# intuitive-robots/mdt_policy

Hardware: AMD Instinct MI355X
Metric: action-chunks/sec (10-step denoise, horizon=10) (higher is better)
Workload: dtype f32

## Files before the change

### include/mdt_hip_ops.h

```cpp
#ifndef MDT_HIP_OPS_H
#define MDT_HIP_OPS_H

#include <stdint.h>
#include "mdt_hip.h"

#ifdef __cplusplus
extern "C" {
#endif

enum { MDT_ACT_NONE = 0, MDT_ACT_GELU = 1, MDT_ACT_MISH = 2, MDT_ACT_SILU = 3,
       MDT_ACT_SWIGLU = 4  };
enum { MDT_HEAD_DENOISED = 0, MDT_HEAD_DDIM = 1, MDT_HEAD_RAW = 2,
       MDT_HEAD_PLAN = 3  };

int64_t mdt_op_packed_numel(int64_t N, int64_t K);

mdt_status mdt_op_pack_weight(const float *w, int64_t n_rows, int64_t K, float *packed, int64_t n_off,
                              int64_t N_total, void *stream);
mdt_status mdt_op_pack_weight_glu(const float *w, int64_t H2, int64_t K, float *packed, void *stream);

typedef struct {
    const float *A;
    int64_t lda;
    const float *Wp;
    const float *bias;
    float *out;
    int64_t ldo;
    int32_t M, N, K;
    int32_t ln;
    const float *ln_w, *ln_b;
    const float *mod;
    int64_t mod_stride;
    int32_t shift_off, scale_off;
    int32_t rows_per_sample;
    int32_t act;
    int32_t residual;
    int32_t gate_off;
    int32_t gin, gout, goff;
    const float *rowvec;
    int32_t batch;
    int64_t bs_a, bs_w, bs_out;
    const float *aux;
    int32_t aux_mode;
    int32_t a_parts;
    int64_t a_part_stride;
    float *a_merged;
    const void *Wp_split;
} mdt_gemm_args;

mdt_status mdt_op_gemm(const mdt_gemm_args *args, void *stream);

mdt_status mdt_op_mlp(const mdt_gemm_args *fc, const mdt_gemm_args *proj, float *parts, int64_t part_stride,
                      int32_t *n_parts, void *stream);
mdt_status mdt_op_pack_weight_split(const float *w, int64_t n_rows, int64_t K, void *image, void *stream);
mdt_status mdt_op_pack_weight_split_rows(const float *w, int64_t n_rows, int64_t K, void *image, int64_t n_off, void *stream);
mdt_status mdt_op_mlp_split(const mdt_gemm_args *fc, const mdt_gemm_args *proj, const void *fc_split, const void *proj_split,
                            float *parts, int64_t part_stride, int32_t *n_parts, void *stream);
void mdt_op_set_mlp_split(int32_t on);
void mdt_op_set_mlp_fuse_min(int32_t rows);
void mdt_op_set_side_jobs(int32_t on);
int64_t mdt_op_side_jobs_paired(void);
void mdt_op_trace_mlp(int32_t enable);
int32_t mdt_op_trace_mlp_read(float *us, int32_t cap);
int32_t mdt_op_trace_mlp_read_empty(float *us, int32_t cap);
mdt_status mdt_op_clock_stamp(uint64_t *out16, void *stream);
void mdt_op_set_ws_split(int32_t on);

void mdt_op_set_mlp_skew(int32_t v);

void mdt_op_set_gemm_geometry(int32_t geometry);

typedef struct {
    const float *q; int64_t ldq;
    const float *k; const float *v;
    int64_t ldkv;
    float *out; int64_t ldo;
    int32_t B, H, hd, Tq, Tk;
    int32_t causal;
    int32_t rope;
} mdt_attn_args;

mdt_status mdt_op_attention(const mdt_attn_args *args, void *stream);

mdt_status mdt_op_attn_proj(const mdt_gemm_args *proj, const float *qkv, int64_t ldq, int32_t hd, int32_t T, int32_t causal,
                            void *stream);
void mdt_op_set_attn_wide_min(int32_t rows);

mdt_status mdt_op_layernorm(const float *in, const float *w, const float *b, float *out, int64_t M, int32_t D,
                            void *stream);

typedef struct {
    const float *y;
    const float *ln_w;
    const float *ln_b;
    const float *Wp, *bp;
    const float *x;
    const float *sigma;
    int64_t sigma_stride;
    float *out;
    int32_t M, D, A, rows_per_sample;
    int32_t mode;
    const float *step;
    float sigma_data;
    float *y_next;
    const float *Wa, *ba;
    int32_t no_ln;
    int32_t y_parts;
    int64_t y_part_stride;
} mdt_head_args;

mdt_status mdt_op_head(const mdt_head_args *args, void *stream);

typedef struct {
    const float *kv; int64_t ldkv;
    const float *WqT_p;
    const float *bq;
    const float *Wo_p;
    float *U, *Wf;
    float *c;
    int32_t B, H, hd, D, Te;
} mdt_xfold_args;
// ... 26 lines not shown
```

### mdt_policy_amd/_lib.py

```python
from __future__ import annotations

import ctypes as C
import os
import threading

from . import build as _build

c_float_p = C.POINTER(C.c_float)


class MDTHipError(RuntimeError):
    def __init__(self, status: int, message: str):
        super().__init__(f"libmdt_hip status {status}: {message}")
        self.status = status


class MDTConfig(C.Structure):
    _fields_ = [(n, C.c_int32) for n in (
        "arch", "embed_dim", "n_heads", "n_enc_layers", "n_dec_layers", "action_dim", "obs_dim", "goal_dim",
        "n_obs_token", "goal_seq_len", "action_seq_len", "use_mlp_goal", "use_modality_encoder", "use_abs_pos_emb",
        "use_rot_embed", "use_ada_conditioning", "use_noise_encoder", "linear_output", "bias")] + [
        ("sigma_data", C.c_float), ("no_goal_conditioning", C.c_int32), ("proprio_dim", C.c_int32),
        ("use_proprio", C.c_int32)]

# ... 155 lines not shown
_VP, _I32, _I64, _F = C.c_void_p, C.c_int32, C.c_int64, C.c_float
SYMBOLS = [
    ("mdt_last_error", C.c_char_p, []),
    ("mdt_version", C.c_char_p, []),
    ("mdt_set_allocator", _I32, [_VP, _VP, _VP]),
    ("mdt_allocator_detach", _I32, []),
    ("mdt_create", _I32, [C.POINTER(MDTConfig), C.POINTER(_VP)]),
    ("mdt_destroy", _I32, [_VP]),
    ("mdt_param_count", _I64, [_VP]),
    ("mdt_param_name", C.c_char_p, [_VP, _I64]),
    ("mdt_param_numel", _I64, [_VP, _I64]),
    ("mdt_load_param", _I32, [_VP, C.c_char_p, _VP, _I64, _VP]),
    ("mdt_load_params", _I32, [_VP, _I32, C.POINTER(C.c_char_p), C.POINTER(C.c_void_p), C.POINTER(_I64), _VP]),
    ("mdt_reserve", _I32, [_VP, _I64]),
    ("mdt_ws_generation", _I64, [_VP]),
    ("mdt_encode", _I32, [_VP, _VP, _VP, _VP, _I32, _I32, _VP, _I64, _VP, _VP]),
    ("mdt_denoise_cached", _I32, [_VP, _VP, _VP, _I64, _I32, _VP, _VP]),
    ("mdt_forward", _I32, [_VP, _VP, _VP, _VP, _I32, _VP, _VP, _I64, _VP, _VP, _VP]),
    ("mdt_sample_ddim", _I32, [_VP, _VP, _VP, _VP, _I32, _VP, C.POINTER(C.c_float), _I32, _I64, _VP, _VP, _VP]),
    ("mdt_sample_ddim_dev", _I32, [_VP, _VP, _VP, _VP, _I32, _VP, _VP, _I32, _I64, _VP, _VP, _VP]),
    ("mdt_sample", _I32, [_VP, _VP, _VP, _VP, _I32, _VP, _I32, C.POINTER(SamplerParams), C.POINTER(C.c_float), _I32, _VP, _I32,
                          _I64, _VP, _VP, _VP]),
    ("mdt_sample_dev", _I32, [_VP, _VP, _VP, _VP, _I32, _VP, _I32, C.POINTER(SamplerParams), _VP, _I32, _VP, _I32, _I64, _VP,
                              _VP, _VP]),
    ("mdt_sampler_plan", _I32, [_I32, C.POINTER(SamplerParams), C.POINTER(C.c_float), _I32, C.POINTER(SamplerPlan)]),
    ("mdt_sample_dpm_adaptive", _I32, [_VP, _VP, _VP, _VP, _I32, _VP, C.c_float, C.c_float, C.POINTER(DpmAdaptiveParams), _I64,
                                       _VP, _VP, C.POINTER(DpmAdaptiveInfo), _VP]),
    ("mdt_dpm_control_init", _I32, [C.POINTER(DpmControl)] + [C.c_double] * 6),
    ("mdt_dpm_control_update", _I32, [C.POINTER(DpmControl), C.c_float, C.POINTER(C.c_int32)]),
    ("mdt_dpm_adaptive_plan", _I32, [_I32, C.c_float, C.c_float, C.POINTER(SamplerPlan)]),
    ("mdt_op_trace_mlp", None, [_I32]),
    ("mdt_op_trace_mlp_read", _I32, [_VP, _I32]),
    ("mdt_op_trace_mlp_read_empty", _I32, [_VP, _I32]),
    ("mdt_op_clock_stamp", _I32, [_VP, _VP]),
    ("mdt_op_set_ws_split", None, [_I32]),
    ("mdt_op_set_tn_split", None, [_I32]),
    ("mdt_loss_fwd", _I32, [_VP, _VP, _VP, _VP, _I32, _VP, _VP, _VP, _I64, _VP, _VP, _VP, _VP]),
    ("mdt_flops_per_chunk", C.c_double, [_VP, _I32]),
    ("mdt_fnv1_32", C.c_uint32, [C.c_char_p, C.c_uint64, C.c_uint32]),
    ("mdt_op_packed_numel", _I64, [_I64, _I64]),
    ("mdt_op_pack_weight", _I32, [_VP, _I64, _I64, _VP, _I64, _I64, _VP]),
    ("mdt_op_pack_weight_glu", _I32, [_VP, _I64, _I64, _VP, _VP]),
    ("mdt_op_gemm", _I32, [C.POINTER(GemmArgs), _VP]),
    ("mdt_op_mlp", _I32, [C.POINTER(GemmArgs), C.POINTER(GemmArgs), _VP, _I64, C.POINTER(_I32), _VP]),
    ("mdt_op_pack_weight_split", _I32, [_VP, _I64, _I64, _VP, _VP]),
    ("mdt_op_pack_weight_split_rows", _I32, [_VP, _I64, _I64, _VP, _I64, _VP]),
    ("mdt_op_mlp_split", _I32, [C.POINTER(GemmArgs), C.POINTER(GemmArgs), _VP, _VP, _VP, _I64, C.POINTER(_I32), _VP]),
    ("mdt_op_set_mlp_split", None, [_I32]),
    ("mdt_op_set_gemm_geometry", None, [_I32]),
    ("mdt_op_set_mlp_fuse_min", None, [_I32]),
    ("mdt_op_set_side_jobs", None, [_I32]),
    ("mdt_op_side_jobs_paired", _I64, []),
    ("mdt_op_set_mlp_skew", None, [_I32]),
    ("mdt_op_set_attn_wide_min", None, [_I32]),
    ("mdt_op_attention", _I32, [C.POINTER(AttnArgs), _VP]),
    ("mdt_op_attn_proj", _I32, [C.POINTER(GemmArgs), _VP, _I64, _I32, _I32, _I32, _VP]),
    ("mdt_op_xattn_fold", _I32, [C.POINTER(XFoldArgs), _VP]),
    ("mdt_op_xattn_apply", _I32, [C.POINTER(XApplyArgs), _VP]),
    ("mdt_op_attn_xattn", _I32, [C.POINTER(GemmArgs), _VP, _I64, C.POINTER(XApplyArgs), _I32, _I32, _VP]),
    ("mdt_op_xattn_gemm", _I32, [C.POINTER(XApplyArgs), C.POINTER(GemmArgs), _VP]),
    ("mdt_op_layernorm", _I32, [_VP, _VP, _VP, _VP, _I64, _I32, _VP]),
    ("mdt_op_head", _I32, [C.POINTER(HeadArgs), _VP]),
    ("mdt_op_action_embed", _I32, [_VP, _VP, _I64, _F, _VP, _VP, _VP, _I64, _I32, _I32, _I32, _VP]),
    ("mdt_train_prepare", _I32, [_VP]),
    ("mdt_grad_numel", _I64, [_VP]),
    ("mdt_grad_offset", _I64, [_VP, _I64]),
    ("mdt_train_loss_fwd", _I32, [_VP, _VP, _VP, _VP, _I32, _VP, _VP, _VP, _I64, C.POINTER(Dropout), _VP, _VP, _VP,
                                  C.POINTER(_I32), _VP]),
    ("mdt_train_loss_bwd", _I32, [_VP, _I32, _VP, _VP, _VP, _VP, _VP, _VP, _VP]),
    ("mdt_train_loss_bwd_stages", _I32, [_VP]),
    ("mdt_train_loss_bwd_stage", _I32, [_VP, _I32, _I32, _VP, _VP, _VP, _VP, _VP, _VP, _VP]),
    ("mdt_train_param_stage", _I32, [_VP, _I64]),
    ("mdt_train_encode_fwd", _I32, [_VP, _VP, _VP, _VP, _I32, _I32, _VP, _I64, C.POINTER(Dropout), _VP, C.POINTER(_I32),
                                    _VP]),
    ("mdt_train_encode_bwd", _I32, [_VP, _I32, _VP, _VP, _VP, _VP, _VP, _VP]),
    ("mdt_tape_release", _I32, [_VP, _I32]),
    ("mdt_denoise_vjp", _I32, [_VP, _VP, _VP, _VP, _I32, _VP, _VP, _VP, _I64, _VP, _VP, _VP]),
    ("mdt_op_pack_weight_t", _I32, [_VP, _I64, _I64, _I64, _VP, _I64, _I64, _VP]),
    ("mdt_op_pack_many", _I32, [_I32, C.POINTER(C.c_void_p), C.POINTER(_I32), C.POINTER(_I32), C.POINTER(C.c_void_p),
                                C.POINTER(C.c_void_p), _VP]),
    ("mdt_op_ln_fwd_train", _I32, [C.POINTER(LnTrainArgs), _VP]),
    ("mdt_op_ln_bwd", _I32, [C.POINTER(LnBwdArgs), _VP]),
    ("mdt_op_attn_bwd", _I32, [C.POINTER(AttnBwdArgs), _VP]),
    ("mdt_op_act_fwd", _I32, [_VP, _VP, _I64, _I32, _VP]),
    ("mdt_op_act_bwd", _I32, [_VP, _VP, _VP, _I64, _I32, _VP]),
    ("mdt_op_attn_fwd_train", _I32, [C.POINTER(AttnTrainArgs), _VP]),
    ("mdt_op_merge_fwd", _I32, [C.POINTER(MergeArgs), _VP]),
    ("mdt_op_merge_bwd", _I32, [C.POINTER(MergeArgs), _VP]),
    ("mdt_op_merge_ln_fwd", _I32, [C.POINTER(MergeArgs), C.POINTER(LnTrainArgs), _VP]),
    ("mdt_op_ln_bwd_merge", _I32, [C.POINTER(LnBwdArgs), C.POINTER(MergeArgs), _VP]),
    ("mdt_op_colsum", _I32, [_VP, _I64, _I64, _I64, _VP, _I32, _VP]),
    ("mdt_op_linear_bwd", _I32, [C.POINTER(LinearBwdArgs), _VP]),
    ("mdt_op_linear_bwd_scratch", _I64, [_I64, _I64, _I64]),
    ("mdt_op_linear_bwd_scratch_exact", _I64, [_I64, _I64, _I64]),
    ("mdt_op_multi_adamw", _I32, [C.POINTER(OptTensor), _I32, _F, _F, _F, _F, _F, _I64, _VP]),
    ("mdt_op_multi_ema", _I32, [C.POINTER(OptTensor), _I32, _F, _VP]),
    ("mdt_resampler_create", _I32, [C.POINTER(ResamplerConfig), C.POINTER(_VP)]),
    ("mdt_resampler_destroy", _I32, [_VP]),
    ("mdt_resampler_param_count", _I64, [_VP]),
    ("mdt_resampler_param_name", C.c_char_p, [_VP, _I64]),
    ("mdt_resampler_param_numel", _I64, [_VP, _I64]),
    ("mdt_resampler_load_param", _I32, [_VP, C.c_char_p, _VP, _I64, _VP]),
    ("mdt_resampler_forward", _I32, [_VP, _VP, _VP, _I64, _I32, _I32, _VP, _VP]),
    ("mdt_resampler_train_prepare", _I32, [_VP]),
    ("mdt_resampler_grad_numel", _I64, [_VP]),
    ("mdt_resampler_grad_offset", _I64, [_VP, _I64]),
# ... 138 lines not shown
```

### mdt_policy_amd/csrc/mdt_kernels.hip

```cpp
#include <hip/hip_runtime.h>

#include <atomic>
#include <stdint.h>
#include <stdlib.h>

#include <mutex>
#include <vector>

#include "mdt_internal.h"

#include "mdt_device.h"

#define MDT_TILES_TIMING_OWNER
#include "mdt_tiles.h"
#include "mdt_sampler_plan.h"
#include "mdt_tall.h"
#include "mdt_ws.h"
#include "mdt_mlp_split.h"

__global__ void k_pack_weight(const float* __restrict__ w, int n_rows, int K, float* __restrict__ packed,
                              int n_off, int K16) {
    const int64_t idx = (int64_t)blockIdx.x * blockDim.x + threadIdx.x;
    if (idx >= (int64_t)n_rows * K) return;
    const int n = (int)(idx / K), k = (int)(idx % K);
// ... 112 lines not shown
            }
        }
    }
}
hipError_t mdt_launch_multi_load(const mdt_load_entry* tab, const int2* blocks, int n_blocks, hipStream_t s) {
    if (n_blocks < 1) return hipSuccess;
    hipLaunchKernelGGL(k_multi_load, dim3(n_blocks), dim3(256), 0, s, tab, blocks);
    return hipGetLastError();
}

#ifdef MDT_DEBUG_TIMING
extern "C" int mdt_debug_set_timing_buffer(unsigned long long* p) {
    return (int)hipMemcpyToSymbol(HIP_SYMBOL(g_dbg_ts), &p, sizeof(p));
}
#endif

template <int MTILES, int NTW, int NWAVES, int PRO, bool RES>
__global__ __launch_bounds__(64 * NWAVES) void k_gemm(mdt_gemm_args a, int kchunk, int grid_n,
                                                      const float* __restrict__ zeros) {
    extern __shared__ __attribute__((aligned(16))) float lds[];
    if (blockIdx.z) {
        a.A += (int64_t)blockIdx.z * a.bs_a; a.Wp += (int64_t)blockIdx.z * a.bs_w; a.out += (int64_t)blockIdx.z * a.bs_out;
    }
    const int logical = xcd_remap(blockIdx.x, gridDim.x);
    const int by = logical / grid_n, bx = logical - by * grid_n;
    gemm_tile<MTILES, NTW, NWAVES, PRO, RES, false>(a, kchunk, by, bx, lds, zeros, threadIdx.x);
}

template <int MTILES, int NTW, int NWAVES, int GLU>
__global__ __launch_bounds__(64 * NWAVES) void k_gemm_glu(mdt_gemm_args a, int kchunk, int grid_n, const float* __restrict__ zeros) {
    extern __shared__ __attribute__((aligned(16))) float lds[];
    const int logical = xcd_remap(blockIdx.x, gridDim.x);
    const int by = logical / grid_n, bx = logical - by * grid_n;
    gemm_tile<MTILES, NTW, NWAVES, PRO_PLAIN, false, false, 1, GLU>(a, kchunk, by, bx, lds, zeros, threadIdx.x);
}

template <int NTW, int PRO, int XP>
__global__ __launch_bounds__(512) void k_gemm_merge(mdt_gemm_args a, int kchunk, int grid_n, const float* __restrict__ zeros) {
    extern __shared__ __attribute__((aligned(16))) float lds[];
    const int logical = xcd_remap(blockIdx.x, gridDim.x);
    const int by = logical / grid_n, bx = logical - by * grid_n;
    gemm_tile<2, NTW, 8, PRO, false, false, XP>(a, kchunk, by, bx, lds, zeros, threadIdx.x);
}

template <int NTW2, int PRO>
__global__ __launch_bounds__(512) void k_mlp(mdt_gemm_args f, mdt_gemm_args p, float* __restrict__ parts, int64_t part_stride,
                                             int n_slices, const float* __restrict__ zeros, int skew) {
    extern __shared__ __attribute__((aligned(16))) float lds[];
    const int logical = xcd_remap(blockIdx.x, gridDim.x);
    const int by = logical / n_slices, s = logical - by * n_slices;
    mlp_tile<NTW2, PRO>(f, p, parts, part_stride, by, s, lds, zeros, threadIdx.x, skew);
}

template <int NTW2, int PRO>
__global__ __launch_bounds__(512) void k_mlp_split(mdt_gemm_args f, mdt_gemm_args p, const char* __restrict__ w1s, const char* __restrict__ w2s,
                                                   float* __restrict__ parts, int64_t part_stride, int n_slices, int gm,
                                                   const float* __restrict__ zeros) {
    extern __shared__ __attribute__((aligned(16))) char lds_c[];
    const int total = gm * n_slices, per = (total + 7) >> 3;
    const int i = blockIdx.x >> 3, w = (blockIdx.x & 7) * per + i;
    if (i >= per || w >= total) return;
    const int s = w / gm, by = w - s * gm;
    mlp_split_tile<NTW2, PRO>(f, p, w1s, w2s, parts, part_stride, by, s, lds_c, zeros, threadIdx.x);
}

template <int MTILES, int NTW, int NWAVES, int LW, bool RES>
__global__ __launch_bounds__(64 * (NWAVES + LW)) void k_gemm_pipe(mdt_gemm_args a, int kchunk, int grid_n,
                                                                 const float* __restrict__ zeros) {
    extern __shared__ __attribute__((aligned(16))) float lds[];
    constexpr int MT = MTILES * 16;
    constexpr bool KSTEP_PRIO = true;
    constexpr int R = NTW == 1 ? 6 : (NTW == 2 ? 4 : 3);
    const f32x4 zero4 = (f32x4){0.f, 0.f, 0.f, 0.f};
    const int tid = threadIdx.x, lane = tid & 63, wave = tid >> 6;
    const bool loader = wave >= NWAVES;
    if (blockIdx.z) {
        a.A += (int64_t)blockIdx.z * a.bs_a; a.Wp += (int64_t)blockIdx.z * a.bs_w; a.out += (int64_t)blockIdx.z * a.bs_out;
    }
    const int logical = xcd_remap(blockIdx.x, gridDim.x);
    const int by = logical / grid_n, bx = logical - by * grid_n;
    const int m0 = by * MT;
    const int N16 = a.N >> 4, K16 = a.K >> 4;
    const int nt0 = (bx * NWAVES + min(wave, NWAVES - 1)) * NTW;
    const bool active = !loader && nt0 < N16;
    const int stride = kchunk + 4;
    const int bufsz = MT * stride;
    const int nchunks = (a.K + kchunk - 1) / kchunk;

    auto stage = [&](int c) {
        constexpr int RG = 2 * LW, U = MT / RG;
        const int lt = tid - 64 * NWAVES, rg = lt >> 5, l32 = lt & 31;
        const int k0 = c * kchunk, n4 = min(kchunk, a.K - k0) >> 2;
        float* dst = lds + (c & 1) * bufsz;
        f32x4 st[U][3];
#pragma unroll
        for (int u = 0; u < U; ++u) {
            const int64_t m = min(m0 + rg + RG * u, a.M - 1);
#pragma unroll
            for (int v = 0; v < 3; ++v) st[u][v] = ldg4(a.A + m * a.lda + k0 + 4 * min(l32 + 32 * v, n4 - 1));
        }
#pragma unroll
        for (int u = 0; u < U; ++u) {
            const int row = rg + RG * u;
#pragma unroll
            for (int v = 0; v < 3; ++v)
                if (l32 + 32 * v < n4) *(f32x4*)(dst + row * stride + 4 * (l32 + 32 * v)) = sel4(m0 + row < a.M, st[u][v], zero4);
        }
    };

    WStream wp[NTW];
    f32x4 ring[R][NTW];
    f32x4 acc[MTILES][NTW];
    const int nq = 4 * (lane >> 4);
    const bool gated = RES && a.gate_off >= 0;
    int ncol[NTW];
    constexpr int NRES = RES ? NTW : 1;
// ... 676 lines not shown
    switch (f.K / 128) {
        case 1: return launch_mlp_pro<1>(f, p, parts, part_stride, s);
        case 2: return launch_mlp_pro<2>(f, p, parts, part_stride, s);
        case 3: return launch_mlp_pro<3>(f, p, parts, part_stride, s);
        default: return launch_mlp_pro<4>(f, p, parts, part_stride, s);
    }
}

template <int ND, int NTW, int PRO, int XP>
__global__ __launch_bounds__(512) void k_gemm_ln_split(mdt_gemm_args a, int grid_n, const float* __restrict__ zeros) {
    extern __shared__ __attribute__((aligned(16))) char lds_c[];
    const int logical = xcd_remap(blockIdx.x, gridDim.x);
    const int by = logical / grid_n, bx = logical - by * grid_n;
    gemm_ln_split_tile<ND, NTW, PRO, XP>(a, by, bx, lds_c, zeros, threadIdx.x);
}
template <int ND, int NTW, int PRO, int XP>
static hipError_t launch_gemm_ln_split_t(const mdt_gemm_args& a, hipStream_t s) {
    const int gn = a.N / (8 * NTW * 16), gm = (a.M + 31) / 32;
    const int lds = 3 * 32 * (2 * 128 * ND + 32);
    static bool attr_dev[MAX_DEVICES] = {false};
    bool& done = attr_dev[current_device()];
    if (!done) {
        hipError_t e = hipFuncSetAttribute((const void*)k_gemm_ln_split<ND, NTW, PRO, XP>, hipFuncAttributeMaxDynamicSharedMemorySize, lds);
        if (e != hipSuccess) return e;
        done = true;
    }
    hipLaunchKernelGGL((k_gemm_ln_split<ND, NTW, PRO, XP>), dim3(gn * gm), dim3(512), lds, s, a, gn, g_zeros);
    return hipGetLastError();
}
template <int ND, int NTW, int PRO>
static hipError_t launch_gemm_ln_split_x(const mdt_gemm_args& a, hipStream_t s) {
    switch (a.a_parts) {
        case 2: return launch_gemm_ln_split_t<ND, NTW, PRO, 2>(a, s);
        case 3: return launch_gemm_ln_split_t<ND, NTW, PRO, 3>(a, s);
        case 4: return launch_gemm_ln_split_t<ND, NTW, PRO, 4>(a, s);
        default: return launch_gemm_ln_split_t<ND, NTW, PRO, 1>(a, s);
    }
}
template <int ND, int NTW>
static hipError_t launch_gemm_ln_split_pro(const mdt_gemm_args& a, hipStream_t s) {
    if (a.mod != nullptr && a.shift_off >= 0)
        return a.mod_stride == 0 ? launch_gemm_ln_split_x<ND, NTW, PRO_LN_MOD_BCAST>(a, s) : launch_gemm_ln_split_x<ND, NTW, PRO_LN_MOD_ROWS>(a, s);
    return launch_gemm_ln_split_x<ND, NTW, PRO_LN>(a, s);
}
static bool gemm_ln_split_applies(const mdt_gemm_args& a) {
    return a.Wp_split != nullptr && mdt_mlp_split_enabled() && a.ln && (a.K == 384 || a.K == 512) && a.N % 384 == 0 &&
           a.M >= mdt_split_min_rows() && a.batch <= 1 && !a.residual && a.gin == 1 && a.gout == 1 && a.goff == 0 && a.rowvec == nullptr && !a.aux_mode &&
           a.a_parts <= 4 && (a.lda & 3) == 0 && (a.ldo & 3) == 0 && g_mdt_gemm_force == 0;
}
static hipError_t launch_gemm_ln_split(const mdt_gemm_args& a, hipStream_t s) {
    return a.K == 512 ? launch_gemm_ln_split_pro<4, 3>(a, s) : launch_gemm_ln_split_pro<3, 3>(a, s);
}

static int g_mlp_split = -1;
bool mdt_mlp_split_enabled() {
    if (g_mlp_split < 0) { const char* e = getenv("MDT_HIP_MLP_SPLIT"); g_mlp_split = e ? atoi(e) : 1; }
    return g_mlp_split != 0;
}
extern "C" void mdt_op_set_mlp_split(int32_t on) { g_mlp_split = on < 0 ? -1 : (on != 0); }
int mdt_split_min_rows() { return 768; }
bool mdt_mlp_split_supported(const mdt_gemm_args& f, const mdt_gemm_args& p) {
    return mdt_mlp_supported(f, p);
}
template <int NTW2, int PRO>
static hipError_t launch_mlp_split_t(const mdt_gemm_args& f, const mdt_gemm_args& p, const void* w1s, const void* w2s, float* parts,
                                     int64_t part_stride, hipStream_t s) {
    const int S = mdt_mlp_slices(f.K), gm = (f.M + 31) / 32;
    const int lds = mlp_split_lds_bytes(128 * NTW2);
    static bool attr_dev[MAX_DEVICES] = {false};
    bool& done = attr_dev[current_device()];
    if (!done) {
        hipError_t e = hipFuncSetAttribute((const void*)k_mlp_split<NTW2, PRO>, hipFuncAttributeMaxDynamicSharedMemorySize, lds);
        if (e != hipSuccess) return e;
        done = true;
    }
    const int per = (gm * S + 7) / 8;
    hipLaunchKernelGGL((k_mlp_split<NTW2, PRO>), dim3(8 * per), dim3(512), lds, s, f, p, (const char*)w1s, (const char*)w2s, parts,
                       part_stride, S, gm, g_zeros);
    return hipGetLastError();
}
template <int NTW2>
static hipError_t launch_mlp_split_pro(const mdt_gemm_args& f, const mdt_gemm_args& p, const void* w1s, const void* w2s, float* parts,
                                       int64_t part_stride, hipStream_t s) {
    if (f.mod != nullptr && f.shift_off >= 0)
        return f.mod_stride == 0 ? launch_mlp_split_t<NTW2, PRO_LN_MOD_BCAST>(f, p, w1s, w2s, parts, part_stride, s)
                                 : launch_mlp_split_t<NTW2, PRO_LN_MOD_ROWS>(f, p, w1s, w2s, parts, part_stride, s);
    return launch_mlp_split_t<NTW2, PRO_LN>(f, p, w1s, w2s, parts, part_stride, s);
}
hipError_t mdt_launch_mlp_split(const mdt_gemm_args& f, const mdt_gemm_args& p, const void* w1s, const void* w2s, float* parts,
                                int64_t part_stride, hipStream_t s) {
    if (!mdt_mlp_split_supported(f, p) || !w1s || !w2s) return hipErrorInvalidValue;
    hipError_t ze = ensure_zeros();
    if (ze != hipSuccess) return ze;
    switch (f.K / 128) {
        case 1: return launch_mlp_split_pro<1>(f, p, w1s, w2s, parts, part_stride, s);
        case 2: return launch_mlp_split_pro<2>(f, p, w1s, w2s, parts, part_stride, s);
        case 3: return launch_mlp_split_pro<3>(f, p, w1s, w2s, parts, part_stride, s);
        default: return launch_mlp_split_pro<4>(f, p, w1s, w2s, parts, part_stride, s);
    }
}

template <int NTW, int PRO, int XP>
static hipError_t launch_gemm_merge_t(const mdt_gemm_args& a, hipStream_t s) {
    const int NTC = 8 * NTW * 16;
    const int gn = (a.N + NTC - 1) / NTC, gm = (a.M + 31) / 32;
    const size_t lds = (size_t)32 * (a.K + 4) * sizeof(float);
    static size_t lds_attr_dev[MAX_DEVICES] = {0};
    size_t& lds_attr = lds_attr_dev[current_device()];
    if (lds > lds_attr) {
        hipError_t e = hipFuncSetAttribute((const void*)k_gemm_merge<NTW, PRO, XP>, hipFuncAttributeMaxDynamicSharedMemorySize, (int)lds);
        if (e != hipSuccess) return e;
        lds_attr = lds;
    }
    hipLaunchKernelGGL((k_gemm_merge<NTW, PRO, XP>), dim3(gn * gm), dim3(512), lds, s, a, a.K, gn, g_zeros);
    return hipGetLastError();
}
template <int NTW, int PRO>
static hipError_t launch_gemm_merge_x(const mdt_gemm_args& a, hipStream_t s) {
    switch (a.a_parts) {
        case 2: return launch_gemm_merge_t<NTW, PRO, 2>(a, s);
        case 3: return launch_gemm_merge_t<NTW, PRO, 3>(a, s);
        case 4: return launch_gemm_merge_t<NTW, PRO, 4>(a, s);
        default: return hipErrorInvalidValue;
    }
}
template <int NTW>
static hipError_t launch_gemm_merge_pro(const mdt_gemm_args& a, hipStream_t s) {
    if (a.mod != nullptr && a.shift_off >= 0)
        return a.mod_stride == 0 ? launch_gemm_merge_x<NTW, PRO_LN_MOD_BCAST>(a, s) : launch_gemm_merge_x<NTW, PRO_LN_MOD_ROWS>(a, s);
    return launch_gemm_merge_x<NTW, PRO_LN>(a, s);
}
static hipError_t launch_gemm_merge(const mdt_gemm_args& a, hipStream_t s) {
// ... 784 lines not shown
```

### mdt_policy_amd/csrc/mdt_mlp_split.h

```cpp
#pragma once
#include <hip/hip_runtime.h>
#include <stdint.h>

#include "mdt_device.h"
#include "mdt_internal.h"
#include "mdt_tiles.h"
#include "mdt_ws.h"

template <int NT, int R>
struct SplitRing {
    mdt_bf16x8 w[R][NT][3];
    __amdgpu_buffer_rsrc_t rs;
    unsigned voff[NT];
    __device__ __forceinline__ void open(const void* image, int64_t first_byte, int64_t tile_stride, int lane) {
        rs = __builtin_amdgcn_make_buffer_rsrc((void*)image, 0, 0xffffffffu, 0x00020000);
#pragma unroll
        for (int j = 0; j < NT; ++j) voff[j] = (unsigned)(first_byte + j * tile_stride) + 16u * (unsigned)lane;
    }
    __device__ __forceinline__ void request(int slot, int kk) {
#pragma unroll
        for (int j = 0; j < NT; ++j)
#pragma unroll
            for (int p = 0; p < 3; ++p)
                w[slot][j][p] = __builtin_bit_cast(mdt_bf16x8, __builtin_amdgcn_raw_buffer_load_b128(rs, voff[j], (kk * 3 + p) * 1024, 0));
    }
};

template <int NT, int K32, int R>
__device__ __forceinline__ void split_phase(SplitRing<NT, R>& ring, const char* xa, int rowb, int part, int lane, f32x4 (&acc)[2][NT]) {
    const int aoff = (lane & 15) * rowb + (lane >> 4) * 16;
    mdt_bf16x8 x1[2], x2[2], x3[2];
#pragma unroll
    for (int i = 0; i < 2; ++i) {
        const char* q = xa + aoff + i * 16 * rowb;
        x1[i] = *(const mdt_bf16x8*)q; x2[i] = *(const mdt_bf16x8*)(q + part); x3[i] = *(const mdt_bf16x8*)(q + 2 * part);
    }
#pragma unroll
    for (int kk = 0; kk < K32; ++kk) {
        const int u = kk % R, un = (kk + R - 1) % R;
        const bool nx = kk + 1 < K32;
        if (kk + R - 1 < K32) ring.request(un, kk + R - 1);
        const char* p0 = xa + aoff + (kk + 1) * 64;
        const char* p1 = p0 + 16 * rowb;
        MDT_SCHED_PIN
#pragma unroll
        for (int j = 0; j < NT; ++j) {
            acc[0][j] = __builtin_amdgcn_mfma_f32_16x16x32_bf16(ring.w[u][j][0], x3[0], acc[0][j], 0, 0, 0);
            acc[1][j] = __builtin_amdgcn_mfma_f32_16x16x32_bf16(ring.w[u][j][0], x3[1], acc[1][j], 0, 0, 0);
        }
        MDT_SCHED_PIN
        if (nx) { x3[0] = *(const mdt_bf16x8*)(p0 + 2 * part); x3[1] = *(const mdt_bf16x8*)(p1 + 2 * part); }
        MDT_SCHED_PIN
#pragma unroll
        for (int j = 0; j < NT; ++j) {
            acc[0][j] = __builtin_amdgcn_mfma_f32_16x16x32_bf16(ring.w[u][j][1], x2[0], acc[0][j], 0, 0, 0);
            acc[1][j] = __builtin_amdgcn_mfma_f32_16x16x32_bf16(ring.w[u][j][1], x2[1], acc[1][j], 0, 0, 0);
        }
#pragma unroll
        for (int j = 0; j < NT; ++j) {
            acc[0][j] = __builtin_amdgcn_mfma_f32_16x16x32_bf16(ring.w[u][j][0], x2[0], acc[0][j], 0, 0, 0);
            acc[1][j] = __builtin_amdgcn_mfma_f32_16x16x32_bf16(ring.w[u][j][0], x2[1], acc[1][j], 0, 0, 0);
        }
        MDT_SCHED_PIN
        if (nx) { x2[0] = *(const mdt_bf16x8*)(p0 + part); x2[1] = *(const mdt_bf16x8*)(p1 + part); }
        MDT_SCHED_PIN
#pragma unroll
        for (int j = 0; j < NT; ++j) {
            acc[0][j] = __builtin_amdgcn_mfma_f32_16x16x32_bf16(ring.w[u][j][2], x1[0], acc[0][j], 0, 0, 0);
            acc[1][j] = __builtin_amdgcn_mfma_f32_16x16x32_bf16(ring.w[u][j][2], x1[1], acc[1][j], 0, 0, 0);
        }
#pragma unroll
        for (int j = 0; j < NT; ++j) {
            acc[0][j] = __builtin_amdgcn_mfma_f32_16x16x32_bf16(ring.w[u][j][1], x1[0], acc[0][j], 0, 0, 0);
            acc[1][j] = __builtin_amdgcn_mfma_f32_16x16x32_bf16(ring.w[u][j][1], x1[1], acc[1][j], 0, 0, 0);
        }
#pragma unroll
        for (int j = 0; j < NT; ++j) {
            acc[0][j] = __builtin_amdgcn_mfma_f32_16x16x32_bf16(ring.w[u][j][0], x1[0], acc[0][j], 0, 0, 0);
            acc[1][j] = __builtin_amdgcn_mfma_f32_16x16x32_bf16(ring.w[u][j][0], x1[1], acc[1][j], 0, 0, 0);
        }
        MDT_SCHED_PIN
        if (nx) { x1[0] = *(const mdt_bf16x8*)p0; x1[1] = *(const mdt_bf16x8*)p1; }
        MDT_SCHED_PIN
    }
}

__host__ __device__ constexpr int mlp_split_lds_bytes(int D) {
    const int xs = 3 * 32 * (2 * D + 32), hs = 3 * 32 * (2 * 512 + 32);
    return xs > hs ? xs : hs;
}

template <int NTW2, int PRO>
__device__ __forceinline__ void mlp_split_tile(const mdt_gemm_args& f, const mdt_gemm_args& p, const char* __restrict__ w1s,
                                               const char* __restrict__ w2s, float* __restrict__ parts, int64_t part_stride, int by,
                                               int s, char* lds, const float* __restrict__ zeros, int tid) {
    constexpr int MTILES = 2, NWAVES = 8, MT = 32, HS = 512, NTW1 = 4, R = 2;
    constexpr int D = 128 * NTW2, K32a = D / 32, K32b = HS / 32;
    constexpr int ROWB1 = 2 * D + 32, PART1 = MT * ROWB1, ROWB2 = 2 * HS + 32, PART2 = MT * ROWB2;
    static_assert(NTW2 >= 1 && NTW2 <= 4, "D <= 512");
    const f32x4 zero4 = (f32x4){0.f, 0.f, 0.f, 0.f};
    const int lane = tid & 63, wave = tid >> 6;
    const int m0 = by * MT;
    const int nq = 4 * (lane >> 4);
    char* xs = lds;
    char* hs = lds;

    const int nt1 = (s * NWAVES + wave) * NTW1;
    SplitRing<NTW1, R> ring1;
    ring1.open(w1s, (int64_t)nt1 * K32a * 3072, (int64_t)K32a * 3072, lane);
#pragma unroll
    for (int u = 0; u < R - 1; ++u) ring1.request(u, u);
    f32x4 b1[NTW1];
    {
        const float* bp = f.bias != nullptr ? f.bias : zeros;
#pragma unroll
        for (int j = 0; j < NTW1; ++j) b1[j] = ldg4(bp + (nt1 + j) * 16 + nq);
    }
    gemm_stage_tile<MTILES, NWAVES, PRO, false, 1, 2, true>(f, (float*)xs, ROWB1, m0, 0, D, zeros, tid, lane, wave);
    __syncthreads();
    f32x4 acc1[MTILES][NTW1];
#pragma unroll
    for (int i = 0; i < MTILES; ++i)
#pragma unroll
        for (int j = 0; j < NTW1; ++j) acc1[i][j] = zero4;
    split_phase<NTW1, K32a, R>(ring1, xs, ROWB1, PART1, lane, acc1);

    const int K32p = p.K >> 5;
    SplitRing<NTW2, R> ring2;
    ring2.open(w2s, ((int64_t)(wave * NTW2) * K32p + (int64_t)s * K32b) * 3072, (int64_t)K32p * 3072, lane);
#pragma unroll
    for (int u = 0; u < R - 1; ++u) ring2.request(u, u);
    constexpr bool EARLY = NTW2 <= 3;
    f32x4 acc2[MTILES][NTW2], b2[NTW2], gate_v[MTILES][NTW2], res_v[MTILES][NTW2];
    int ncol[NTW2];
#pragma unroll
    for (int j = 0; j < NTW2; ++j) ncol[j] = (wave * NTW2 + j) * 16 + nq;
    const bool gated = p.mod != nullptr && p.gate_off >= 0;
    auto load_gate_res = [&]() __attribute__((always_inline)) {
#pragma unroll
        for (int i = 0; i < MTILES; ++i) {
            const int64_t m = min(m0 + i * 16 + (lane & 15), f.M - 1);
            const float* gp = gated ? p.mod + p.gate_off + (p.mod_stride == 0 ? 0 : (m / p.rows_per_sample) * p.mod_stride)
                                    : zeros;
            const float* rp = s == 0 ? f.A + m * f.lda : zeros;
#pragma unroll
            for (int j = 0; j < NTW2; ++j) {
                gate_v[i][j] = ldg4(gp + ncol[j]);
                res_v[i][j] = ldg4(rp + ncol[j]);
            }
        }
    };
    {
        const float* bp = (s == 0 && p.bias != nullptr) ? p.bias : zeros;
#pragma unroll
        for (int j = 0; j < NTW2; ++j) b2[j] = ldg4(bp + ncol[j]);
#pragma unroll
        for (int i = 0; i < MTILES; ++i)
#pragma unroll
            for (int j = 0; j < NTW2; ++j) acc2[i][j] = zero4;
        if constexpr (EARLY) load_gate_res();
    }
    __syncthreads();
#pragma unroll
    for (int i = 0; i < MTILES; ++i)
#pragma unroll
        for (int j = 0; j < NTW1; ++j) {
            mdt_bf16x4 p1, p2, p3;
            split3_bf16(apply_act(acc1[i][j] + b1[j], f.act), p1, p2, p3);
            char* q = hs + split_slot(i * 16 + (lane & 15), (wave * NTW1 + j) * 16 + nq, ROWB2);
            *(mdt_bf16x4*)q = p1;
            *(mdt_bf16x4*)(q + PART2) = p2;
            *(mdt_bf16x4*)(q + 2 * PART2) = p3;
        }
    __syncthreads();
    split_phase<NTW2, K32b, R>(ring2, hs, ROWB2, PART2, lane, acc2);

    if constexpr (!EARLY) load_gate_res();
    float* out = parts + (int64_t)s * part_stride;
#pragma unroll
    for (int i = 0; i < MTILES; ++i) {
        const int m = m0 + i * 16 + (lane & 15);
#pragma unroll
        for (int j = 0; j < NTW2; ++j) {
            f32x4 v = acc2[i][j] + b2[j];
            v = res_v[i][j] + (gated ? gate_v[i][j] * v : v);
            if (m < f.M) st4(out + (int64_t)m * p.ldo + ncol[j], v);
        }
    }
}

template <int ND, int NTW, int PRO, int XP>
__device__ __forceinline__ void gemm_ln_split_tile(const mdt_gemm_args& a, int by, int bx, char* lds, const float* __restrict__ zeros, int tid) {
    constexpr int MTILES = 2, NWAVES = 8, MT = 32, R = 2;
    constexpr int D = 128 * ND, K32 = D / 32, ROWB = 2 * D + 32, PART = MT * ROWB;
    static_assert(ND >= 1 && ND <= 4, "D <= 512");
    const f32x4 zero4 = (f32x4){0.f, 0.f, 0.f, 0.f};
    const int lane = tid & 63, wave = tid >> 6;
    const int m0 = by * MT, nq = 4 * (lane >> 4);
    char* xs = lds;
    const int nt0 = (bx * NWAVES + wave) * NTW;
    SplitRing<NTW, R> ring;
    ring.open(a.Wp_split, (int64_t)nt0 * K32 * 3072, (int64_t)K32 * 3072, lane);
#pragma unroll
    for (int u = 0; u < R - 1; ++u) ring.request(u, u);
    f32x4 bias_v[NTW];
    {
        const float* bp = a.bias != nullptr ? a.bias : zeros;
#pragma unroll
        for (int j = 0; j < NTW; ++j) bias_v[j] = ldg4(bp + (nt0 + j) * 16 + nq);
    }
    gemm_stage_tile<MTILES, NWAVES, PRO, false, XP, (NTW <= 3 && XP <= 3) ? 1 : 2, true>(a, (float*)xs, ROWB, m0, 0, D, zeros, tid, lane, wave,
                                                                                         bx == 0 ? a.a_merged : nullptr);
    __syncthreads();
    f32x4 acc[MTILES][NTW];
#pragma unroll
    for (int i = 0; i < MTILES; ++i)
#pragma unroll
        for (int j = 0; j < NTW; ++j) acc[i][j] = zero4;
    split_phase<NTW, K32, R>(ring, xs, ROWB, PART, lane, acc);
#pragma unroll
    for (int i = 0; i < MTILES; ++i) {
        const int m = m0 + i * 16 + (lane & 15);
#pragma unroll
        for (int j = 0; j < NTW; ++j)
            if (m < a.M) st4(a.out + (int64_t)m * a.ldo + (nt0 + j) * 16 + nq, apply_act(acc[i][j] + bias_v[j], a.act));
    }
}
```

Baseline: 74770.

## Replace block barriers in split MLP with per-wave LDS flags and skewed waves

The split-weight MLP tile now staggers its waves. The late half waits on LDS flags set by the early half partway through the first GEMM, and the second GEMM consumes hidden-activation chunks as soon as their producing waves flag them, instead of waiting at __syncthreads. The hidden buffer is split into two separate regions so it no longer aliases the input staging buffer while skewed waves are still reading it. An optional s_setprio boost, on by default, is also added. The aim is to remove barrier stalls and spread out memory and MFMA pressure, at the cost of extra LDS, spin-wait flags, and more template instantiations.

```diff
diff --git a/include/mdt_hip_ops.h b/include/mdt_hip_ops.h
--- a/include/mdt_hip_ops.h
+++ b/include/mdt_hip_ops.h
@@ -67,6 +67,8 @@
 void mdt_op_set_ws_split(int32_t on);
 
 void mdt_op_set_mlp_skew(int32_t v);
+
+void mdt_op_set_mlp_split_skew(int32_t v);
 
 void mdt_op_set_gemm_geometry(int32_t geometry);
 
diff --git a/mdt_policy_amd/_lib.py b/mdt_policy_amd/_lib.py
--- a/mdt_policy_amd/_lib.py
+++ b/mdt_policy_amd/_lib.py
@@ -231,6 +231,7 @@
     ("mdt_op_set_side_jobs", None, [_I32]),
     ("mdt_op_side_jobs_paired", _I64, []),
     ("mdt_op_set_mlp_skew", None, [_I32]),
+    ("mdt_op_set_mlp_split_skew", None, [_I32]),
     ("mdt_op_set_attn_wide_min", None, [_I32]),
     ("mdt_op_attention", _I32, [C.POINTER(AttnArgs), _VP]),
     ("mdt_op_attn_proj", _I32, [C.POINTER(GemmArgs), _VP, _I64, _I32, _I32, _I32, _VP]),
diff --git a/mdt_policy_amd/csrc/mdt_kernels.hip b/mdt_policy_amd/csrc/mdt_kernels.hip
--- a/mdt_policy_amd/csrc/mdt_kernels.hip
+++ b/mdt_policy_amd/csrc/mdt_kernels.hip
@@ -188,16 +188,16 @@
     mlp_tile<NTW2, PRO>(f, p, parts, part_stride, by, s, lds, zeros, threadIdx.x, skew);
 }
 
-template <int NTW2, int PRO>
+template <int NTW2, int PRO, int SKEW>
 __global__ __launch_bounds__(512) void k_mlp_split(mdt_gemm_args f, mdt_gemm_args p, const char* __restrict__ w1s, const char* __restrict__ w2s,
                                                    float* __restrict__ parts, int64_t part_stride, int n_slices, int gm,
-                                                   const float* __restrict__ zeros) {
+                                                   const float* __restrict__ zeros, int prio) {
     extern __shared__ __attribute__((aligned(16))) char lds_c[];
     const int total = gm * n_slices, per = (total + 7) >> 3;
     const int i = blockIdx.x >> 3, w = (blockIdx.x & 7) * per + i;
     if (i >= per || w >= total) return;
     const int s = w / gm, by = w - s * gm;
-    mlp_split_tile<NTW2, PRO>(f, p, w1s, w2s, parts, part_stride, by, s, lds_c, zeros, threadIdx.x);
+    mlp_split_tile<NTW2, PRO, SKEW>(f, p, w1s, w2s, parts, part_stride, by, s, lds_c, zeros, threadIdx.x, prio != 0);
 }
 
 template <int MTILES, int NTW, int NWAVES, int LW, bool RES>
@@ -980,6 +980,7 @@
     return a.K == 512 ? launch_gemm_ln_split_pro<4, 3>(a, s) : launch_gemm_ln_split_pro<3, 3>(a, s);
 }
 
+#define MDT_MLP_SPLIT_SKEW_DEFAULT (8 | 256)
 static int g_mlp_split = -1;
 bool mdt_mlp_split_enabled() {
     if (g_mlp_split < 0) { const char* e = getenv("MDT_HIP_MLP_SPLIT"); g_mlp_split = e ? atoi(e) : 1; }
@@ -990,22 +991,41 @@
 bool mdt_mlp_split_supported(const mdt_gemm_args& f, const mdt_gemm_args& p) {
     return mdt_mlp_supported(f, p);
 }
-template <int NTW2, int PRO>
+static int g_mlp_split_skew = -1;
+static int mlp_split_skew() { return g_mlp_split_skew < 0 ? MDT_MLP_SPLIT_SKEW_DEFAULT : g_mlp_split_skew; }
+extern "C" void mdt_op_set_mlp_split_skew(int32_t v) { g_mlp_split_skew = v < 0 ? -1 : (v & 0x1ff); }
+
+template <int NTW2, int PRO, int SKEW>
 static hipError_t launch_mlp_split_t(const mdt_gemm_args& f, const mdt_gemm_args& p, const void* w1s, const void* w2s, float* parts,
-                                     int64_t part_stride, hipStream_t s) {
+                                     int64_t part_stride, int prio, hipStream_t s) {
     const int S = mdt_mlp_slices(f.K), gm = (f.M + 31) / 32;
     const int lds = mlp_split_lds_bytes(128 * NTW2);
     static bool attr_dev[MAX_DEVICES] = {false};
     bool& done = attr_dev[current_device()];
     if (!done) {
-        hipError_t e = hipFuncSetAttribute((const void*)k_mlp_split<NTW2, PRO>, hipFuncAttributeMaxDynamicSharedMemorySize, lds);
+        hipError_t e = hipFuncSetAttribute((const void*)k_mlp_split<NTW2, PRO, SKEW>, hipFuncAttributeMaxDynamicSharedMemorySize, lds);
         if (e != hipSuccess) return e;
         done = true;
     }
     const int per = (gm * S + 7) / 8;
-    hipLaunchKernelGGL((k_mlp_split<NTW2, PRO>), dim3(8 * per), dim3(512), lds, s, f, p, (const char*)w1s, (const char*)w2s, parts,
-                       part_stride, S, gm, g_zeros);
-    return hipGetLastError();
+    hipLaunchKernelGGL((k_mlp_split<NTW2, PRO, SKEW>), dim3(8 * per), dim3(512), lds, s, f, p, (const char*)w1s, (const char*)w2s, parts,
+                       part_stride, S, gm, g_zeros, prio);
+    return hipGetLastError();
+}
+template <int NTW2, int PRO, int SKEW = 4 * NTW2>
+static hipError_t launch_mlp_split_skew(const mdt_gemm_args& f, const mdt_gemm_args& p, const void* w1s, const void* w2s, float* parts,
+                                        int64_t part_stride, int skew, int prio, hipStream_t s) {
+    if constexpr (SKEW > 0) {
+        if (skew < SKEW) return launch_mlp_split_skew<NTW2, PRO, SKEW - 2>(f, p, w1s, w2s, parts, part_stride, skew, prio, s);
+    }
+    return launch_mlp_split_t<NTW2, PRO, SKEW>(f, p, w1s, w2s, parts, part_stride, prio, s);
+}
+template <int NTW2, int PRO>
+static hipError_t launch_mlp_split_t(const mdt_gemm_args& f, const mdt_gemm_args& p, const void* w1s, const void* w2s, float* parts,
+                                     int64_t part_stride, hipStream_t s) {
+    const int v = mlp_split_skew();
+    const int skew = min(v & 0xff, 4 * NTW2) & ~1;
+    return launch_mlp_split_skew<NTW2, PRO>(f, p, w1s, w2s, parts, part_stride, skew, (v & 0x100) ? 1 : 0, s);
 }
 template <int NTW2>
 static hipError_t launch_mlp_split_pro(const mdt_gemm_args& f, const mdt_gemm_args& p, const void* w1s, const void* w2s, float* parts,
diff --git a/mdt_policy_amd/csrc/mdt_mlp_split.h b/mdt_policy_amd/csrc/mdt_mlp_split.h
--- a/mdt_policy_amd/csrc/mdt_mlp_split.h
+++ b/mdt_policy_amd/csrc/mdt_mlp_split.h
@@ -26,21 +26,35 @@
     }
 };
 
-template <int NT, int K32, int R>
-__device__ __forceinline__ void split_phase(SplitRing<NT, R>& ring, const char* xa, int rowb, int part, int lane, f32x4 (&acc)[2][NT]) {
+template <int KH>
+__device__ __forceinline__ const char* split_step_src(const char* xa, const char* xb, int kk) {
+    return kk < KH ? xa + kk * 64 : xb + (kk - KH) * 64;
+}
+template <int KH>
+__device__ __forceinline__ void split_load_step(const char* xa, const char* xb, int rowb, int part, int lane, int kk, mdt_bf16x8 (&x1)[2],
+                                                mdt_bf16x8 (&x2)[2], mdt_bf16x8 (&x3)[2]) {
+    const char* q0 = split_step_src<KH>(xa, xb, kk) + (lane & 15) * rowb + (lane >> 4) * 16;
+#pragma unroll
+    for (int i = 0; i < 2; ++i) {
+        const char* q = q0 + i * 16 * rowb;
+        x1[i] = *(const mdt_bf16x8*)q; x2[i] = *(const mdt_bf16x8*)(q + part); x3[i] = *(const mdt_bf16x8*)(q + 2 * part);
+    }
+}
+struct SplitNoPre {
+    __device__ __forceinline__ void operator()(int) const {}
+};
+template <int NT, int K32, int R, int KB, int KE, int KH = K32, class Pre = SplitNoPre>
+__device__ __forceinline__ void split_steps(SplitRing<NT, R>& ring, const char* xa, const char* xb, int rowb, int part, int lane,
+                                            mdt_bf16x8 (&x1)[2], mdt_bf16x8 (&x2)[2], mdt_bf16x8 (&x3)[2], f32x4 (&acc)[2][NT],
+                                            const Pre& pre = Pre()) {
     const int aoff = (lane & 15) * rowb + (lane >> 4) * 16;
-    mdt_bf16x8 x1[2], x2[2], x3[2];
-#pragma unroll
-    for (int i = 0; i < 2; ++i) {
-        const char* q = xa + aoff + i * 16 * rowb;
-        x1[i] = *(const mdt_bf16x8*)q; x2[i] = *(const mdt_bf16x8*)(q + part); x3[i] = *(const mdt_bf16x8*)(q + 2 * part);
-    }
-#pragma unroll
-    for (int kk = 0; kk < K32; ++kk) {
+#pragma unroll
+    for (int kk = KB; kk < KE; ++kk) {
         const int u = kk % R, un = (kk + R - 1) % R;
         const bool nx = kk + 1 < K32;
         if (kk + R - 1 < K32) ring.request(un, kk + R - 1);
-        const char* p0 = xa + aoff + (kk + 1) * 64;
+        pre(kk);
+        const char* p0 = split_step_src<KH>(xa, xb, nx ? kk + 1 : kk) + aoff;
         const char* p1 = p0 + 16 * rowb;
         MDT_SCHED_PIN
 #pragma unroll
@@ -85,25 +99,49 @@
     }
 }
 
-__host__ __device__ constexpr int mlp_split_lds_bytes(int D) {
-    const int xs = 3 * 32 * (2 * D + 32), hs = 3 * 32 * (2 * 512 + 32);
-    return xs > hs ? xs : hs;
-}
-
-template <int NTW2, int PRO>
+template <int NT, int K32, int R>
+__device__ __forceinline__ void split_phase(SplitRing<NT, R>& ring, const char* xa, int rowb, int part, int lane, f32x4 (&acc)[2][NT]) {
+    mdt_bf16x8 x1[2], x2[2], x3[2];
+    split_load_step<K32>(xa, xa, rowb, part, lane, 0, x1, x2, x3);
+    split_steps<NT, K32, R, 0, K32>(ring, xa, xa, rowb, part, lane, x1, x2, x3, acc);
+}
+
+constexpr int MLPS_ROWH = 2 * 256 + 32, MLPS_PARTH = 32 * MLPS_ROWH, MLPS_REGION = 3 * MLPS_PARTH;
+__host__ __device__ constexpr int mlp_split_region_a(int D) {
+    return 3 * 32 * (2 * D + 32) > MLPS_REGION ? 3 * 32 * (2 * D + 32) : MLPS_REGION;
+}
+__host__ __device__ constexpr int mlp_split_flags(int D) { return mlp_split_region_a(D) + MLPS_REGION; }
+__host__ __device__ constexpr int mlp_split_lds_bytes(int D) { return mlp_split_flags(D) + 32 * 4; }
+
+__device__ __forceinline__ void mlp_wait_all8(const int* flg) {
+    unsigned ready = 0;
+#pragma unroll 1
+    for (int c = 0; c < 8; ++c) mlp_wait_chunk(flg, c, ready);
+}
+
+template <int NTW2, int PRO, int SKEW>
 __device__ __forceinline__ void mlp_split_tile(const mdt_gemm_args& f, const mdt_gemm_args& p, const char* __restrict__ w1s,
                                                const char* __restrict__ w2s, float* __restrict__ parts, int64_t part_stride, int by,
-                                               int s, char* lds, const float* __restrict__ zeros, int tid) {
+                                               int s, char* lds, const float* __restrict__ zeros, int tid, bool prio) {
     constexpr int MTILES = 2, NWAVES = 8, MT = 32, HS = 512, NTW1 = 4, R = 2;
-    constexpr int D = 128 * NTW2, K32a = D / 32, K32b = HS / 32;
-    constexpr int ROWB1 = 2 * D + 32, PART1 = MT * ROWB1, ROWB2 = 2 * HS + 32, PART2 = MT * ROWB2;
+    constexpr int D = 128 * NTW2, K32a = D / 32, K32b = HS / 32, K32h = K32b / 2;
+    constexpr int ROWB1 = 2 * D + 32, PART1 = MT * ROWB1, ROWB2 = MLPS_ROWH, PART2 = MLPS_PARTH;
     static_assert(NTW2 >= 1 && NTW2 <= 4, "D <= 512");
+    static_assert(SKEW >= 0 && SKEW <= K32a && SKEW % R == 0, "skew in whole ring rounds, inside the first product");
+    static_assert(mlp_split_lds_bytes(D) <= 163840, "LDS");
+    constexpr bool SKEWED = SKEW > 0;
     const f32x4 zero4 = (f32x4){0.f, 0.f, 0.f, 0.f};
     const int lane = tid & 63, wave = tid >> 6;
     const int m0 = by * MT;
     const int nq = 4 * (lane >> 4);
+    const bool late = wave >= NWAVES / 2;
     char* xs = lds;
-    char* hs = lds;
+    char* hb = lds;
+    char* ha = lds + mlp_split_region_a(D);
+    int* flg = (int*)(lds + mlp_split_flags(D));
+    if constexpr (SKEWED) {
+        if (tid < 32) flg[tid] = 0;
+    }
 
     const int nt1 = (s * NWAVES + wave) * NTW1;
     SplitRing<NTW1, R> ring1;
@@ -123,7 +161,20 @@
     for (int i = 0; i < MTILES; ++i)
 #pragma unroll
         for (int j = 0; j < NTW1; ++j) acc1[i][j] = zero4;
-    split_phase<NTW1, K32a, R>(ring1, xs, ROWB1, PART1, lane, acc1);
+    {
+        mdt_bf16x8 x1[2], x2[2], x3[2];
+        split_load_step<K32a>(xs, xs, ROWB1, PART1, lane, 0, x1, x2, x3);
+        if (SKEWED && late) mlp_wait_flag(flg + 16 + (wave & 3));
+        if (prio) __builtin_amdgcn_s_setprio(2);
+        split_steps<NTW1, K32a, R, 0, SKEW>(ring1, xs, xs, ROWB1, PART1, lane, x1, x2, x3, acc1);
+        if (SKEWED && !late) mlp_set_flag(flg + 16 + (wave & 3), lane);
+        split_steps<NTW1, K32a, R, SKEW, K32a>(ring1, xs, xs, ROWB1, PART1, lane, x1, x2, x3, acc1);
+        if (prio) __builtin_amdgcn_s_setprio(0);
+    }
+    if constexpr (SKEWED) {
+        asm volatile("s_waitcnt lgkmcnt(0)" ::: "memory");
+        mlp_set_flag(flg + 8 + wave, lane);
+    }
 
     const int K32p = p.K >> 5;
     SplitRing<NTW2, R> ring2;
@@ -160,20 +211,48 @@
             for (int j = 0; j < NTW2; ++j) acc2[i][j] = zero4;
         if constexpr (EARLY) load_gate_res();
     }
-    __syncthreads();
-#pragma unroll
-    for (int i = 0; i < MTILES; ++i)
-#pragma unroll
-        for (int j = 0; j < NTW1; ++j) {
-            mdt_bf16x4 p1, p2, p3;
-            split3_bf16(apply_act(acc1[i][j] + b1[j], f.act), p1, p2, p3);
-            char* q = hs + split_slot(i * 16 + (lane & 15), (wave * NTW1 + j) * 16 + nq, ROWB2);
-            *(mdt_bf16x4*)q = p1;
-            *(mdt_bf16x4*)(q + PART2) = p2;
-            *(mdt_bf16x4*)(q + 2 * PART2) = p3;
-        }
-    __syncthreads();
-    split_phase<NTW2, K32b, R>(ring2, hs, ROWB2, PART2, lane, acc2);
+    if constexpr (SKEWED) {
+        if (late) mlp_wait_all8(flg + 8);
+    } else {
+        __syncthreads();
+    }
+    {
+        char* hr = late ? hb : ha;
+        const int c0 = (wave & 3) * NTW1 * 16;
+#pragma unroll
+        for (int i = 0; i < MTILES; ++i)
+#pragma unroll
+            for (int j = 0; j < NTW1; ++j) {
+                mdt_bf16x4 p1, p2, p3;
+                split3_bf16(apply_act(acc1[i][j] + b1[j], f.act), p1, p2, p3);
+                char* q = hr + split_slot(i * 16 + (lane & 15), c0 + j * 16 + nq, ROWB2);
+                *(mdt_bf16x4*)q = p1;
+                *(mdt_bf16x4*)(q + PART2) = p2;
+                *(mdt_bf16x4*)(q + 2 * PART2) = p3;
+            }
+    }
+    {
+        mdt_bf16x8 x1[2], x2[2], x3[2];
+        if constexpr (SKEWED) {
+            asm volatile("s_waitcnt lgkmcnt(0)" ::: "memory");
+            mlp_set_flag(flg + wave, lane);
+            unsigned ready = 0;
+            mlp_wait_chunk(flg, 0, ready);
+            split_load_step<K32h>(ha, hb, ROWB2, PART2, lane, 0, x1, x2, x3);
+            if (prio) __builtin_amdgcn_s_setprio(2);
+            auto pre = [&](int kk) __attribute__((always_inline)) {
+                if (((kk + 1) & 1) == 0 && kk + 1 < K32b) mlp_wait_chunk(flg, (kk + 1) >> 1, ready);
+            };
+            split_steps<NTW2, K32b, R, 0, K32b, K32h>(ring2, ha, hb, ROWB2, PART2, lane, x1, x2, x3, acc2, pre);
+            if (prio) __builtin_amdgcn_s_setprio(0);
+        } else {
+            __syncthreads();
+            split_load_step<K32h>(ha, hb, ROWB2, PART2, lane, 0, x1, x2, x3);
+            if (prio) __builtin_amdgcn_s_setprio(2);
+            split_steps<NTW2, K32b, R, 0, K32b, K32h>(ring2, ha, hb, ROWB2, PART2, lane, x1, x2, x3, acc2);
+            if (prio) __builtin_amdgcn_s_setprio(0);
+        }
+    }
 
     if constexpr (!EARLY) load_gate_res();
     float* out = parts + (int64_t)s * part_stride;
```

Measured after the change: 75490 (median of 6 runs). About the same (+1.0%).
